# Shadowfear36/SegHiero

Measured on AMD Instinct MI355X. Metric: images/sec at 512x512 (ResNet-50 2-level), full train step, higher is better.
Workload: dtype f32 (convolutions: exact 3-way bf16 split of every fp32 operand, 6 bf16 MFMA products, f32 accumulate; rest plain f32)

## Files before the change

seghiero_amd/csrc/bn_elementwise.hip:

```cpp
#include "common.h"
#include <stdlib.h>

static inline unsigned grid_for(long long work_items, int block = 256, int cap = 4096) {
    long long g = sh_cdiv(work_items, block);
    if (g > cap) g = cap;
    if (g < 1) g = 1;
    return (unsigned)g;
}

__global__ __launch_bounds__(256) void nchw_to_nhwc_kernel(const float* __restrict__ x, float* __restrict__ y,
                                                           int C, long long HW, int Cpad, long long total) {
    for (long long i = (long long)blockIdx.x * 256 + threadIdx.x; i < total; i += (long long)gridDim.x * 256) {
        const int c = (int)(i % Cpad);
        const long long q = i / Cpad, hw = q % HW, n = q / HW;
        y[i] = c < C ? x[(n * C + c) * HW + hw] : 0.f;
    }
}
__global__ __launch_bounds__(256) void nhwc_to_nchw_kernel(const float* __restrict__ x, float* __restrict__ y,
                                                           int C, long long HW, int Cpad, long long total) {
    for (long long i = (long long)blockIdx.x * 256 + threadIdx.x; i < total; i += (long long)gridDim.x * 256) {
        const long long hw = i % HW, q = i / HW;
        const int c = (int)(q % C);
        const long long n = q / C;
        y[i] = x[(n * HW + hw) * Cpad + c];
// ... 268 lines not shown
        !beta || !running_mean || !running_var || !mean || !invstd || !scale || !shift) return SH_EINVAL;
    if ((long long)n_partials != sh_cdiv((long long)count, rows_per_partial) || (partials_ld != 0 && partials_ld < C)) return SH_EINVAL;
    BnMultiTab T;
    for (int i = 0; i < k; ++i) {
        if (!mean[i] || !invstd[i] || !scale[i] || !shift[i] || partials_col[i] < 0 || (running_mean[i] == nullptr) != (running_var[i] == nullptr))
            return SH_EINVAL;
        T.gamma[i] = gamma[i]; T.beta[i] = beta[i]; T.rm[i] = running_mean[i]; T.rv[i] = running_var[i];
        T.mean[i] = mean[i]; T.invstd[i] = invstd[i]; T.scale[i] = scale[i]; T.shift[i] = shift[i];
        T.wmul[i] = chan_mul ? chan_mul[i] : nullptr; T.isy[i] = isy ? isy[i] : nullptr; T.col[i] = partials_col[i];
        if (T.wmul[i] && chan_stride <= 0) return SH_EINVAL;
    }
    dim3 grid((unsigned)sh_cdiv(C, 4), (unsigned)k);
    bn_finalize_multi_kernel<<<grid, 256, 0, (hipStream_t)stream>>>(partials, n_partials, C, count, eps, momentum, rows_per_partial, partials_ld,
                                                                   chan_stride, T);
    return sh_launch_status();
}
extern "C" int sh_bn_finalize_scaled(const float* partials, int n_partials, int C, double count, const float* chan_mul, int chan_stride,
                                     const float* gamma, const float* beta, float eps, float momentum, float* running_mean,
                                     float* running_var, float* mean, float* invstd, float* scale, float* shift, float* isy,
                                     int rows_per_partial, void* stream) {
    if (!partials || n_partials <= 0 || C <= 0 || count <= 0 || !chan_mul || chan_stride <= 0 || !mean || !invstd || !scale || !shift || !isy ||
        rows_per_partial <= 0) return SH_EINVAL;
    if ((long long)n_partials != sh_cdiv((long long)count, rows_per_partial)) return SH_EINVAL;
    if ((running_mean == nullptr) != (running_var == nullptr)) return SH_EINVAL;
    bn_finalize_kernel<256><<<(unsigned)sh_cdiv(C, 4), 256, 0, (hipStream_t)stream>>>(
        partials, n_partials, C, count, gamma, beta, eps, momentum, running_mean, running_var, mean, invstd, scale, shift, rows_per_partial,
        0, chan_mul, chan_stride, isy);
    return sh_launch_status();
}
__global__ __launch_bounds__(64) void dw_center_wgrad_kernel(const float* __restrict__ dgamma, const float* __restrict__ gamma,
                                                             const float* __restrict__ isy, const float* __restrict__ w, float eps,
                                                             float* __restrict__ dw, int C, const float* __restrict__ g, long long ldg,
                                                             const float* __restrict__ x, long long ldx, const float* __restrict__ mean_x,
                                                             long long M) {
    const int c = blockIdx.x, t = threadIdx.x;
    const float wc = w[(long long)c * 9 + 4];
    const float gm = gamma ? gamma[c] : 1.f;
    float v = 0.f;
    if (wc != 0.f) v = gm * dgamma[c] * eps * isy[c] * isy[c] / wc;
    else if (g != nullptr) {
        const float mu = mean_x[c];
        double s = 0.0;
        for (long long m = t; m < M; m += 64) s += (double)g[m * ldg + c] * (double)(x[m * ldx + c] - mu);
#pragma unroll
        for (int o = 32; o > 0; o >>= 1) s += __shfl_xor(s, o, 64);
        v = (float)((double)gm * (double)isy[c] * s);
    }
    if (t < 9) dw[(long long)c * 9 + t] = t == 4 ? v : 0.f;
}
extern "C" int sh_dw_center_wgrad(const float* dgamma, const float* gamma, const float* isy, const float* w, float eps, float* dw, int C,
                                  const float* g, int ldg, const float* x, int ldx, const float* mean_x, int64_t M, void* stream) {
    if (!dgamma || !isy || !w || !dw || C <= 0) return SH_EINVAL;
    if (g && (!x || !mean_x || ldg < C || ldx < C || M <= 0)) return SH_EINVAL;
    dw_center_wgrad_kernel<<<(unsigned)C, 64, 0, (hipStream_t)stream>>>(dgamma, gamma, isy, w, eps, dw, C, g, ldg, x, ldx, mean_x, M);
    return sh_launch_status();
}

__global__ __launch_bounds__(256) void bn_eval_coefs_kernel(const float* gamma, const float* beta, const float* rm,
                                                            const float* rv, float eps, int C, float* scale, float* shift) {
    const int c = blockIdx.x * 256 + threadIdx.x;
    if (c >= C) return;
    const float is = 1.0f / sqrtf(rv[c] + eps);
    const float sc = (gamma ? gamma[c] : 1.f) * is;
    scale[c] = sc;
    shift[c] = (beta ? beta[c] : 0.f) - rm[c] * sc;
}
extern "C" int sh_bn_eval_coefs(const float* gamma, const float* beta, const float* running_mean,
                                const float* running_var, float eps, int C, float* scale, float* shift, void* stream) {
    if (!running_mean || !running_var || !scale || !shift || C <= 0) return SH_EINVAL;
    bn_eval_coefs_kernel<<<(unsigned)sh_cdiv(C, 256), 256, 0, (hipStream_t)stream>>>(gamma, beta, running_mean, running_var, eps, C, scale, shift);
    return sh_launch_status();
}

#define STAT_ROWS 256
template <int KIND>
__global__ __launch_bounds__(256) void channel_partials_kernel(const float* __restrict__ y, long long ldy,
                                                               const float* __restrict__ dout, long long lddo,
                                                               const float* __restrict__ out, long long ldo,
                                                               const float* __restrict__ mean, const float* __restrict__ invstd,
                                                               const float* __restrict__ scale, const float* __restrict__ shift,
                                                               float* __restrict__ partials, long long M, int C, int relu) {
    __shared__ float red[2][4][64];
    const int t = threadIdx.x, cl = t & 63, g = t >> 6;
    const int c = blockIdx.y * 64 + cl;
    const long long rbeg = (long long)blockIdx.x * STAT_ROWS;
    const long long rend = rbeg + STAT_ROWS < M ? rbeg + STAT_ROWS : M;
    float s = 0.f, q = 0.f;
    if (c < C) {
        float mu = 0.f, is = 0.f, sc = 0.f, sh = 0.f;
        if (KIND == 1) { mu = mean[c]; is = invstd[c]; if (relu == 2) { sc = scale[c]; sh = shift[c]; } }
        for (long long r = rbeg + g; r < rend; r += 4) {
            if (KIND == 0) {
                const float v = y[r * ldy + c];
                s += v; q += v * v;
            } else {
                float gv = dout[r * lddo + c];
                const float yv = y[r * ldy + c];
                if (relu == 1 && !(out[r * ldo + c] > 0.f)) gv = 0.f;
                if (relu == 2 && !(yv * sc + sh > 0.f)) gv = 0.f;
                const float xh = (yv - mu) * is;
                s += gv; q += gv * xh;
            }
        }
    }
    if (KIND == 0) {
        float n = 0.f, mean = 0.f, m2 = 0.f;
        if (c < C)
            for (long long r = rbeg + g; r < rend; r += 4) {
                const float v = y[r * ldy + c];
                n += 1.f;
                const float d = v - mean;
                mean += d / n;
                m2 += d * (v - mean);
            }
        red[0][g][cl] = n * mean; red[1][g][cl] = m2;
        __shared__ float cnt[4][64];
        cnt[g][cl] = n;
        __syncthreads();
        if (t < 64) {
            const int ch = blockIdx.y * 64 + t;
            if (ch < C) {
                float N = cnt[0][t], S = red[0][0][t], Q = red[1][0][t];
#pragma unroll
                for (int k = 1; k < 4; ++k) {
                    const float nb = cnt[k][t], sb = red[0][k][t];
                    if (nb > 0.f) {
                        if (N > 0.f) { const float dm = S / N - sb / nb; Q += red[1][k][t] + dm * dm * N * nb / (N + nb); }
                        else Q = red[1][k][t];
                        N += nb; S += sb;
                    }
                }
                partials[((long long)blockIdx.x * 2 + 0) * C + ch] = S;
                partials[((long long)blockIdx.x * 2 + 1) * C + ch] = Q;
            }
        }
        return;
    }
    red[0][g][cl] = s; red[1][g][cl] = q;
    __syncthreads();
    if (t < 128) {
        const int st = t >> 6, cc = t & 63, ch = blockIdx.y * 64 + cc;
        if (ch < C)
            partials[((long long)blockIdx.x * 2 + st) * C + ch] = (red[st][0][cc] + red[st][1][cc]) + (red[st][2][cc] + red[st][3][cc]);
    }
}
__global__ __launch_bounds__(256) void channel_stats_v4_kernel(const float* __restrict__ y, long long ldy, float* __restrict__ partials,
                                                               long long M, int C) {
    __shared__ float red[16][64];
    __shared__ float colmean[64];
    const int t = threadIdx.x, cq = t & 15, rl = t >> 4;
    const unsigned nch = (unsigned)((C + 63) / 64), rb = blockIdx.x / nch, cb = blockIdx.x % nch;
    const int c = cb * 64 + cq * 4;
    const long long rbeg = (long long)rb * STAT_ROWS;
    const long long left = M - rbeg;
    const float nvalid = (float)(left < STAT_ROWS ? left : STAT_ROWS);
    f32x4 v[STAT_ROWS / 16];
    f32x4 s = {0.f, 0.f, 0.f, 0.f};
#pragma unroll
    for (int k = 0; k < STAT_ROWS / 16; ++k) {
        const long long r = rbeg + rl + 16 * k;
        v[k] = (c < C && r < M) ? ld4(y + r * ldy + c) : f32x4{0.f, 0.f, 0.f, 0.f};
        s += v[k];
    }
#pragma unroll
    for (int j = 0; j < 4; ++j) red[rl][cq * 4 + j] = s[j];
    __syncthreads();
    float colsum = 0.f;
    if (t < 64) {
#pragma unroll
        for (int k = 0; k < 16; ++k) colsum += red[k][t];
        colmean[t] = colsum / nvalid;
    }
    __syncthreads();
    const f32x4 mu = ld4(&colmean[cq * 4]);
    f32x4 q = {0.f, 0.f, 0.f, 0.f};
#pragma unroll
    for (int k = 0; k < STAT_ROWS / 16; ++k)
        if (rbeg + rl + 16 * k < M) { const f32x4 d = v[k] - mu; q += d * d; }
#pragma unroll
    for (int j = 0; j < 4; ++j) red[rl][cq * 4 + j] = q[j];
    __syncthreads();
    if (t < 64 && cb * 64 + t < C) {
        float m2 = 0.f;
#pragma unroll
        for (int k = 0; k < 16; ++k) m2 += red[k][t];
        partials[((long long)rb * 2 + 0) * C + cb * 64 + t] = colsum;
        partials[((long long)rb * 2 + 1) * C + cb * 64 + t] = m2;
    }
}
extern "C" int sh_stats_partials_count(int64_t M) { return (int)sh_cdiv(M, STAT_ROWS); }
extern "C" int sh_stats_tile_rows(void) { return STAT_ROWS; }
extern "C" int sh_channel_stats(const float* y, int ldy, int64_t M, int C, float* partials, void* stream) {
    if (!y || !partials || M <= 0 || C <= 0 || ldy < C) return SH_EINVAL;
    dim3 grid((unsigned)sh_cdiv(M, STAT_ROWS), (unsigned)sh_cdiv(C, 64));
    if ((C & 3) == 0 && (ldy & 3) == 0 && ((uintptr_t)y & 15) == 0)
        channel_stats_v4_kernel<<<grid.x * grid.y, 256, 0, (hipStream_t)stream>>>(y, ldy, partials, M, C);
    else
        channel_partials_kernel<0><<<grid, 256, 0, (hipStream_t)stream>>>(y, ldy, nullptr, 0, nullptr, 0, nullptr, nullptr, nullptr, nullptr, partials, M, C, 0);
    return sh_launch_status();
}
__global__ __launch_bounds__(256) void bn_bwd_partials_v4_kernel(const float* __restrict__ y, long long ldy,
                                                                 const float* __restrict__ dout, long long lddo,
                                                                 const float* __restrict__ out, long long ldo,
                                                                 const float* __restrict__ mean, const float* __restrict__ invstd,
                                                                 const float* __restrict__ scale, const float* __restrict__ shift,
                                                                 float* __restrict__ partials, long long M, int C, int relu,
                                                                 float* __restrict__ g_out, long long ldg, int af) {
    __shared__ float red[2][16][64];
    const int t = threadIdx.x, cq = t & 15, rl = t >> 4;
    const unsigned nch = (unsigned)((C + 63) / 64), rb = blockIdx.x / nch, cb = blockIdx.x % nch;
    const int c = cb * 64 + cq * 4;
    const long long rbeg = (long long)rb * STAT_ROWS;
    f32x4 s = {0.f, 0.f, 0.f, 0.f}, q = {0.f, 0.f, 0.f, 0.f};
    if (c < C) {
        const f32x4 mu = ld4(mean + c), is = ld4(invstd + c);
        f32x4 sc = {0.f, 0.f, 0.f, 0.f}, sh = sc;
        if (relu == 2) { sc = ld4(scale + c); sh = ld4(shift + c); }
#pragma unroll 4
        for (int k = 0; k < STAT_ROWS / 16; ++k) {
            const long long r = rbeg + rl + 16 * k;
            if (r < M) {
                f32x4 g = lda4(dout, r * lddo + c, af & 4);
                const f32x4 yv = lda4(y, r * ldy + c, af & 1);
                if (relu == 1) {
                    const f32x4 o = lda4(out, r * ldo + c, af & 2);
#pragma unroll
                    for (int j = 0; j < 4; ++j) g[j] = o[j] > 0.f ? g[j] : 0.f;
                } else if (relu == 2) {
                    const f32x4 o = yv * sc + sh;
#pragma unroll
                    for (int j = 0; j < 4; ++j) g[j] = o[j] > 0.f ? g[j] : 0.f;
                } else if (relu == 3) {
                    const f32x4 o = quad_mask_load(out, r * ldo + (c >> 2));
#pragma unroll
                    for (int j = 0; j < 4; ++j) g[j] = o[j] > 0.f ? g[j] : 0.f;
                }
                s += g;
                q += g * ((yv - mu) * is);
                if (g_out) sta4(g_out, r * ldg + c, g, af & 8);
            }
        }
    }
#pragma unroll
    for (int j = 0; j < 4; ++j) { red[0][rl][cq * 4 + j] = s[j]; red[1][rl][cq * 4 + j] = q[j]; }
    __syncthreads();
    if (t < 128) {
        const int st = t >> 6, cc = t & 63, ch = cb * 64 + cc;
        if (ch < C) {
            float a = 0.f;
#pragma unroll
            for (int k = 0; k < 16; ++k) a += red[st][k][cc];
            partials[((long long)rb * 2 + st) * C + ch] = a;
        }
    }
}
extern "C" int sh_bn_bwd_reduce(const float* dout, int lddo, const float* out, int ldo, const float* y, int ldy,
                                const float* mean, const float* invstd, const float* scale, const float* shift, float* partials,
                                int64_t M, int C, int relu, float* g_out, int ldg, int act_flags, void* stream) {
    if (!dout || !y || !mean || !invstd || !partials || M <= 0 || C <= 0 || lddo < C || ldy < C) return SH_EINVAL;
    if (g_out && (ldg < C || (ldg & 3) || ((uintptr_t)g_out & 15))) return SH_EINVAL;
    if (relu < 0 || relu > 3 || (relu == 1 && (!out || ldo < C)) || (relu == 2 && (!scale || !shift)) || (relu == 3 && (!out || ldo * 4 < C))) return SH_EINVAL;
    dim3 grid((unsigned)sh_cdiv(M, STAT_ROWS), (unsigned)sh_cdiv(C, 64));
    const bool v4 = (C & 3) == 0 && ((lddo | ldy | (relu == 1 ? ldo : 0)) & 3) == 0 && ((uintptr_t)dout & 15) == 0 && ((uintptr_t)y & 15) == 0 &&
                    (relu != 1 || ((uintptr_t)out & 15) == 0) && ((uintptr_t)mean & 15) == 0 && ((uintptr_t)invstd & 15) == 0 &&
                    (relu != 2 || ((((uintptr_t)scale | (uintptr_t)shift) & 15) == 0));
    if (v4) bn_bwd_partials_v4_kernel<<<grid.x * grid.y, 256, 0, (hipStream_t)stream>>>(y, ldy, dout, lddo, out, ldo, mean, invstd, scale, shift, partials, M, C, relu, g_out, ldg, act_flags);
    else if (g_out || act_flags || relu == 3) return SH_EUNSUPPORTED;
    else channel_partials_kernel<1><<<grid, 256, 0, (hipStream_t)stream>>>(y, ldy, dout, lddo, out, ldo, mean, invstd, scale, shift, partials, M, C, relu);
    return sh_launch_status();
}

__device__ __forceinline__ void bn_bwd_lin(float* lin, int C, int c, float ga, float is, float mu, float c1, float c2) {
    const float A = ga * is;
    lin[c] = A; lin[C + c] = -(A * is) * c2; lin[2 * C + c] = mu; lin[3 * C + c] = -A * c1;
}
template <int NT>
__global__ __launch_bounds__(NT) void bn_bwd_finalize_kernel(const float* __restrict__ partials, int P, int C,
                                                              const float* __restrict__ gamma, const float* __restrict__ invstd,
                                                              double count, float* dgamma, float* dbeta, float* c1, float* c2,
                                                              const float* __restrict__ mean, float* __restrict__ lin) {
    const int cpre = blockIdx.x * 4 + threadIdx.x;
    float ga = 1.f, is = 0.f, mu = 0.f;
    if (lin && threadIdx.x < 4 && cpre < C) { if (gamma) ga = gamma[cpre]; is = invstd[cpre]; mu = mean[cpre]; }
    reduce_partials_4ch<NT>(partials, P, C, blockIdx.x * 4, 0, 0, [&](int c, double s, double q) {
        if (dbeta) dbeta[c] = (float)s;
        if (dgamma) dgamma[c] = (float)q;
        const float f1 = (float)(s / count), f2 = (float)(q / count);
        c1[c] = f1;
        c2[c] = f2;
        if (lin) bn_bwd_lin(lin, C, c, ga, is, mu, f1, f2);
    });
}
extern "C" int sh_bn_bwd_finalize(const float* partials, int n_partials, int C, const float* gamma, const float* invstd,
                                  double count, float* dgamma, float* dbeta, float* c1, float* c2, const float* mean, float* lin,
                                  void* stream) {
    if (!partials || n_partials <= 0 || C <= 0 || count <= 0 || !c1 || !c2 || (lin && (!mean || !invstd))) return SH_EINVAL;
    if (n_partials >= 1024)
        bn_bwd_finalize_kernel<1024><<<(unsigned)sh_cdiv(C, 4), 1024, 0, (hipStream_t)stream>>>(partials, n_partials, C, gamma, invstd, count, dgamma, dbeta, c1, c2, mean, lin);
    else
        bn_bwd_finalize_kernel<256><<<(unsigned)sh_cdiv(C, 4), 256, 0, (hipStream_t)stream>>>(partials, n_partials, C, gamma, invstd, count, dgamma, dbeta, c1, c2, mean, lin);
    return sh_launch_status();
}

#define EW_ROWS 16
template <int V>
__global__ __launch_bounds__(256) void bn_act_kernel(const float* __restrict__ y, long long ldy, const float* __restrict__ scale,
                                                     const float* __restrict__ shift, const float* __restrict__ res, long long ldr,
                                                     float* __restrict__ out, long long ldo, long long M, int C, int relu,
                                                     const float* __restrict__ rscale, const float* __restrict__ rshift, int af,
                                                     unsigned char* __restrict__ qmask) {
    const int cv = C / V;
    for (long long m0 = (long long)blockIdx.x * EW_ROWS; m0 < M; m0 += (long long)gridDim.x * EW_ROWS)
    for (int e = threadIdx.x, tot = (int)((M - m0 < EW_ROWS ? M - m0 : EW_ROWS)) * cv; e < tot; e += 256) {
        const int r = e / cv;
        const long long m = m0 + r;
        const int c = (e - r * cv) * V;
        if (V == 8) {
            const sh_f8 yv = lda8(y, m * ldy + c, af & 1);
            sh_f8 v;
            v.lo = yv.lo * ld4(scale + c) + ld4(shift + c); v.hi = yv.hi * ld4(scale + c + 4) + ld4(shift + c + 4);
            if (res) {
                sh_f8 r = lda8(res, m * ldr + c, af & 2);
                if (rscale) { r.lo = r.lo * ld4(rscale + c) + ld4(rshift + c); r.hi = r.hi * ld4(rscale + c + 4) + ld4(rshift + c + 4); }
                v.lo += r.lo; v.hi += r.hi;
            }
            if (relu) {
#pragma unroll
                for (int j = 0; j < 4; ++j) { v.lo[j] = fmaxf(v.lo[j], 0.f); v.hi[j] = fmaxf(v.hi[j], 0.f); }
            }
            sta8(out, m * ldo + c, v, af & 4);
            if (qmask) *reinterpret_cast<unsigned short*>(qmask + m * (C / 4) + (c >> 2)) = (unsigned short)(quad_mask_bits(v.lo) | (quad_mask_bits(v.hi) << 8));
        } else if (V == 4) {
            f32x4 v = lda4(y, m * ldy + c, af & 1) * ld4(scale + c) + ld4(shift + c);
            if (res) {
                f32x4 r = lda4(res, m * ldr + c, af & 2);
                if (rscale) r = r * ld4(rscale + c) + ld4(rshift + c);
                v += r;
            }
            if (relu) { v[0] = fmaxf(v[0], 0.f); v[1] = fmaxf(v[1], 0.f); v[2] = fmaxf(v[2], 0.f); v[3] = fmaxf(v[3], 0.f); }
            sta4(out, m * ldo + c, v, af & 4);
            if (qmask) qmask[m * cv + (c >> 2)] = (unsigned char)quad_mask_bits(v);
        } else {
            float v = y[m * ldy + c] * scale[c] + shift[c];
            if (res) v += rscale ? res[m * ldr + c] * rscale[c] + rshift[c] : res[m * ldr + c];
            if (relu) v = fmaxf(v, 0.f);
            out[m * ldo + c] = v;
        }
    }
}
static inline unsigned rows_grid(long long M, int cv) {
    (void)cv;
    long long g = sh_cdiv(M, EW_ROWS);
    if (g > 8192) g = 8192;
    return (unsigned)(g < 1 ? 1 : g);
}
static inline bool vec4_ok(int C, long long a, long long b = 0, long long c = 0, long long d = 0, long long e = 0) {
    return (C & 3) == 0 && ((a | b | c | d | e) & 3) == 0;
}
static inline bool ptr16(const void* p) { return ((uintptr_t)p & 15) == 0; }
static inline bool ew8_on() { const char* e = getenv("SEGHIERO_EW8"); return !(e && e[0] == '0'); }

extern "C" int sh_bn_act(const float* y, int ldy, const float* scale, const float* shift, const float* residual, int ldr,
                         const float* res_scale, const float* res_shift, float* out, int ldo, int64_t M, int C, int relu, uint8_t* relu_mask,
                         int act_flags, void* stream) {
    if (!y || !scale || !shift || !out || M <= 0 || C <= 0 || ldy < C || ldo < C) return SH_EINVAL;
    if (residual && ldr < C) return SH_EINVAL;
    if ((res_scale == nullptr) != (res_shift == nullptr) || (res_scale && !residual)) return SH_EINVAL;
    const bool v4 = vec4_ok(C, ldy, ldo, residual ? ldr : 0) && ptr16(y) && ptr16(out) && ptr16(scale) && ptr16(shift) && (!residual || ptr16(residual)) &&
                    (!res_scale || (ptr16(res_scale) && ptr16(res_shift)));
    if ((act_flags || relu_mask) && !v4) return SH_EUNSUPPORTED;
    const bool v8 = v4 && ew8_on() && (act_flags & 1) && (C & 7) == 0 && ((ldy | ldo | (residual ? ldr : 0)) & 7) == 0 && (!relu_mask || ((uintptr_t)relu_mask & 1) == 0);
    if (v8) bn_act_kernel<8><<<rows_grid(M, C / 8), 256, 0, (hipStream_t)stream>>>(y, ldy, scale, shift, residual, ldr, out, ldo, M, C, relu, res_scale, res_shift, act_flags, relu_mask);
    else if (v4) bn_act_kernel<4><<<rows_grid(M, C / 4), 256, 0, (hipStream_t)stream>>>(y, ldy, scale, shift, residual, ldr, out, ldo, M, C, relu, res_scale, res_shift, act_flags, relu_mask);
    else bn_act_kernel<1><<<rows_grid(M, C), 256, 0, (hipStream_t)stream>>>(y, ldy, scale, shift, residual, ldr, out, ldo, M, C, relu, res_scale, res_shift, 0, nullptr);
    return sh_launch_status();
}

template <int V>
__global__ __launch_bounds__(256) void bn_bwd_apply_kernel(const float* __restrict__ dout, long long lddo, const float* __restrict__ out,
                                                           long long ldo, const float* __restrict__ y, long long ldy,
                                                           const float* __restrict__ mean, const float* __restrict__ invstd,
                                                           const float* __restrict__ scale, const float* __restrict__ shift,
                                                           const float* __restrict__ gamma, const float* __restrict__ c1,
                                                           const float* __restrict__ c2, float* __restrict__ dy, long long lddy,
                                                           float* __restrict__ dres, long long lddres, long long M, int C, int relu, int af) {
    const int cv = C / V;
    for (long long m0 = (long long)blockIdx.x * EW_ROWS; m0 < M; m0 += (long long)gridDim.x * EW_ROWS)
    for (int e = threadIdx.x, tot = (int)((M - m0 < EW_ROWS ? M - m0 : EW_ROWS)) * cv; e < tot; e += 256) {
        const int r = e / cv;
        const long long m = m0 + r;
        const int c = (e - r * cv) * V;
        if (V == 8) {
            sh_f8 g8 = lda8(dout, m * lddo + c, af & 4);
            const sh_f8 y8 = lda8(y, m * ldy + c, af & 1);
            sh_f8 o8 = sh_f8{f32x4{1.f, 1.f, 1.f, 1.f}, f32x4{1.f, 1.f, 1.f, 1.f}};
            if (relu == 1) o8 = lda8(out, m * ldo + c, af & 2);
            else if (relu == 2) { o8.lo = y8.lo * ld4(scale + c) + ld4(shift + c); o8.hi = y8.hi * ld4(scale + c + 4) + ld4(shift + c + 4); }
            else if (relu == 3) { o8.lo = quad_mask_load(out, m * ldo + (c >> 2)); o8.hi = quad_mask_load(out, m * ldo + (c >> 2) + 1); }
            if (relu) {
#pragma unroll
                for (int j = 0; j < 4; ++j) { if (!(o8.lo[j] > 0.f)) g8.lo[j] = 0.f; if (!(o8.hi[j] > 0.f)) g8.hi[j] = 0.f; }
            }
            sh_f8 r8;
            {
                const f32x4 is = ld4(invstd + c), xh = (y8.lo - ld4(mean + c)) * is;
                f32x4 ga = {1.f, 1.f, 1.f, 1.f};
                if (gamma) ga = ld4(gamma + c);
                r8.lo = ga * is * (g8.lo - ld4(c1 + c) - xh * ld4(c2 + c));
            }
            {
                const f32x4 is = ld4(invstd + c + 4), xh = (y8.hi - ld4(mean + c + 4)) * is;
                f32x4 ga = {1.f, 1.f, 1.f, 1.f};
                if (gamma) ga = ld4(gamma + c + 4);
                r8.hi = ga * is * (g8.hi - ld4(c1 + c + 4) - xh * ld4(c2 + c + 4));
            }
            sta8(dy, m * lddy + c, r8, af & 8);
            if (dres) sta8(dres, m * lddres + c, g8, af & 16);
        } else if (V == 4) {
            f32x4 g = lda4(dout, m * lddo + c, af & 4);
            const f32x4 yv = lda4(y, m * ldy + c, af & 1);
            if (relu == 1) {
                const f32x4 o = lda4(out, m * ldo + c, af & 2);
#pragma unroll
                for (int j = 0; j < 4; ++j) if (!(o[j] > 0.f)) g[j] = 0.f;
            } else if (relu == 2) {
                const f32x4 o = yv * ld4(scale + c) + ld4(shift + c);
#pragma unroll
                for (int j = 0; j < 4; ++j) if (!(o[j] > 0.f)) g[j] = 0.f;
            } else if (relu == 3) {
                const f32x4 o = quad_mask_load(out, m * ldo + (c >> 2));
#pragma unroll
                for (int j = 0; j < 4; ++j) if (!(o[j] > 0.f)) g[j] = 0.f;
            }
            const f32x4 is = ld4(invstd + c);
            const f32x4 xh = (yv - ld4(mean + c)) * is;
            f32x4 ga = {1.f, 1.f, 1.f, 1.f};
            if (gamma) ga = ld4(gamma + c);
            const f32x4 r = ga * is * (g - ld4(c1 + c) - xh * ld4(c2 + c));
            sta4(dy, m * lddy + c, r, af & 8);
            if (dres) sta4(dres, m * lddres + c, g, af & 16);
        } else {
            float g = dout[m * lddo + c];
            const float yv = y[m * ldy + c];
            if (relu == 1 && !(out[m * ldo + c] > 0.f)) g = 0.f;
            if (relu == 2 && !(yv * scale[c] + shift[c] > 0.f)) g = 0.f;
            const float is = invstd[c];
            const float xh = (yv - mean[c]) * is;
            dy[m * lddy + c] = (gamma ? gamma[c] : 1.f) * is * (g - c1[c] - xh * c2[c]);
            if (dres) dres[m * lddres + c] = g;
        }
    }
}
extern "C" int sh_bn_bwd_apply(const float* dout, int lddo, const float* out, int ldo, const float* y, int ldy,
                               const float* mean, const float* invstd, const float* scale, const float* shift, const float* gamma,
                               const float* c1, const float* c2, float* dy, int lddy, float* dres, int lddres, int64_t M, int C, int relu,
                               int act_flags, void* stream) {
    if (!dout || !y || !mean || !invstd || !c1 || !c2 || !dy || M <= 0 || C <= 0 || lddo < C || ldy < C || lddy < C) return SH_EINVAL;
    if (relu < 0 || relu > 3 || (relu == 1 && (!out || ldo < C)) || (relu == 2 && (!scale || !shift)) || (relu == 3 && (!out || ldo * 4 < C))) return SH_EINVAL;
    if (dres && lddres < C) return SH_EINVAL;
    const bool v4 = vec4_ok(C, lddo, ldy, lddy, relu == 1 ? ldo : 0, dres ? lddres : 0) && ptr16(dout) && ptr16(y) && ptr16(dy) &&
                    ptr16(mean) && ptr16(invstd) && ptr16(c1) && ptr16(c2) && (!gamma || ptr16(gamma)) && (relu != 1 || ptr16(out)) &&
                    (relu != 2 || (ptr16(scale) && ptr16(shift))) && (!dres || ptr16(dres));
    if ((act_flags || relu == 3) && !v4) return SH_EUNSUPPORTED;
    const bool v8 = v4 && ew8_on() && (act_flags & 1) && (C & 7) == 0 && ((lddo | ldy | lddy | (relu == 1 ? ldo : 0) | (dres ? lddres : 0)) & 7) == 0 && (relu != 3 || (ldo & 1) == 0);
    if (v8) bn_bwd_apply_kernel<8><<<rows_grid(M, C / 8), 256, 0, (hipStream_t)stream>>>(dout, lddo, out, ldo, y, ldy, mean, invstd, scale, shift, gamma, c1, c2, dy, lddy, dres, lddres, M, C, relu, act_flags);
    else if (v4) bn_bwd_apply_kernel<4><<<rows_grid(M, C / 4), 256, 0, (hipStream_t)stream>>>(dout, lddo, out, ldo, y, ldy, mean, invstd, scale, shift, gamma, c1, c2, dy, lddy, dres, lddres, M, C, relu, act_flags);
    else bn_bwd_apply_kernel<1><<<rows_grid(M, C), 256, 0, (hipStream_t)stream>>>(dout, lddo, out, ldo, y, ldy, mean, invstd, scale, shift, gamma, c1, c2, dy, lddy, dres, lddres, M, C, relu, 0);
    return sh_launch_status();
}

__global__ __launch_bounds__(256) void bn_reduce_partials_kernel(const float* __restrict__ partials, int P, int C, int R, long long M,
                                                                 double* __restrict__ sq) {
    if (blockIdx.x == 0 && threadIdx.x == 0) sq[2 * C] = (double)M;
    reduce_partials_4ch(partials, P, C, blockIdx.x * 4, R, M, [&](int c, double s, double q) { sq[c] = s; sq[C + c] = q; });
}
extern "C" int sh_bn_reduce_partials(const float* partials, int n_partials, int C, double count, int rows_per_partial, double* sq,
                                     void* stream) {
    if (!partials || !sq || n_partials <= 0 || C <= 0 || rows_per_partial < 0) return SH_EINVAL;
    bn_reduce_partials_kernel<<<(unsigned)sh_cdiv(C, 4), 256, 0, (hipStream_t)stream>>>(partials, n_partials, C, rows_per_partial,
                                                                                       (long long)count, sq);
    return sh_launch_status();
}
__global__ __launch_bounds__(256) void bn_finalize_sq_kernel(const double* __restrict__ sq, int C, const float* __restrict__ gamma,
                                                             const float* __restrict__ beta, float eps, float momentum, float* running_mean,
                                                             float* running_var, float* mean, float* invstd, float* scale, float* shift) {
    const int c = blockIdx.x * 256 + threadIdx.x;
    if (c >= C) return;
    const double count = sq[2 * C];
    const double mu = sq[c] / count;
    double var = sq[C + c] / count - mu * mu;
    if (var < 0) var = 0;
    const float fmu = (float)mu, is = 1.0f / sqrtf((float)var + eps);
    mean[c] = fmu; invstd[c] = is;
    const float sc = (gamma ? gamma[c] : 1.f) * is;
    scale[c] = sc; shift[c] = (beta ? beta[c] : 0.f) - fmu * sc;
    if (running_mean) {
        const double unbiased = count > 1 ? var * (count / (count - 1.0)) : var;
        running_mean[c] = (1.f - momentum) * running_mean[c] + momentum * fmu;
        running_var[c] = (1.f - momentum) * running_var[c] + momentum * (float)unbiased;
    }
}
extern "C" int sh_bn_finalize_sq(const double* sq, int C, const float* gamma, const float* beta, float eps, float momentum,
                                 float* running_mean, float* running_var, float* mean, float* invstd, float* scale, float* shift,
                                 void* stream) {
    if (!sq || C <= 0 || !mean || !invstd || !scale || !shift) return SH_EINVAL;
    bn_finalize_sq_kernel<<<(unsigned)sh_cdiv(C, 256), 256, 0, (hipStream_t)stream>>>(sq, C, gamma, beta, eps, momentum, running_mean,
                                                                                      running_var, mean, invstd, scale, shift);
    return sh_launch_status();
}
__global__ __launch_bounds__(256) void bn_bwd_finalize_sq_kernel(const double* __restrict__ local_sq, const double* __restrict__ global_sq, int C,
                                                                 float* dgamma, float* dbeta, float* c1, float* c2, const float* gamma,
                                                                 const float* invstd, const float* mean, float* lin) {
    const int c = blockIdx.x * 256 + threadIdx.x;
    if (c >= C) return;
    const double count = global_sq[2 * C];
    if (dbeta) dbeta[c] = (float)local_sq[c];
    if (dgamma) dgamma[c] = (float)local_sq[C + c];
    const float f1 = (float)(global_sq[c] / count), f2 = (float)(global_sq[C + c] / count);
    c1[c] = f1;
    c2[c] = f2;
    if (lin) bn_bwd_lin(lin, C, c, gamma ? gamma[c] : 1.f, invstd[c], mean[c], f1, f2);
}
extern "C" int sh_bn_bwd_finalize_sq(const double* local_sq, const double* global_sq, int C, float* dgamma, float* dbeta,
                                     float* c1, float* c2, const float* gamma, const float* invstd, const float* mean, float* lin, void* stream) {
    if (!local_sq || !global_sq || C <= 0 || !c1 || !c2 || (lin && (!mean || !invstd))) return SH_EINVAL;
    bn_bwd_finalize_sq_kernel<<<(unsigned)sh_cdiv(C, 256), 256, 0, (hipStream_t)stream>>>(local_sq, global_sq, C, dgamma, dbeta, c1, c2, gamma, invstd, mean, lin);
    return sh_launch_status();
}
```

seghiero_amd/csrc/common.h:

```cpp
#pragma once
#include <hip/hip_runtime.h>
#include <stdint.h>
#include "../../include/seghiero_hip.h"

typedef float f32x4 __attribute__((ext_vector_type(4)));
typedef float f32x16 __attribute__((ext_vector_type(16)));

#define SH_WAVE 64

static inline int sh_launch_status() {
    hipError_t e = hipGetLastError();
    return e == hipSuccess ? SH_OK : SH_ELAUNCH;
}

static inline int64_t sh_cdiv(int64_t a, int64_t b) { return (a + b - 1) / b; }

__device__ __forceinline__ float wave_sum(float v) {
#pragma unroll
    for (int o = 32; o > 0; o >>= 1) v += __shfl_xor(v, o, 64);
    return v;
}
__device__ __forceinline__ double wave_sum_d(double v) {
#pragma unroll
    for (int o = 32; o > 0; o >>= 1) v += __shfl_xor(v, o, 64);
    return v;
}

__device__ __forceinline__ unsigned xcd_remap(unsigned bid, unsigned nblk) {
    const unsigned q = nblk >> 3, r = nblk & 7u, xcd = bid & 7u, loc = bid >> 3;
    const unsigned base = xcd < r ? xcd * (q + 1) : r * (q + 1) + (xcd - r) * q;
    return base + loc;
}

__device__ __forceinline__ f32x4 ld4(const float* p) { return *reinterpret_cast<const f32x4*>(p); }
__device__ __forceinline__ void st4(float* p, f32x4 v) { *reinterpret_cast<f32x4*>(p) = v; }

typedef unsigned int sh_u32x2 __attribute__((ext_vector_type(2)));
__device__ __forceinline__ f32x4 bf16x4_to_f32(sh_u32x2 v) {
    return f32x4{__uint_as_float(v[0] << 16), __uint_as_float(v[0] & 0xffff0000u), __uint_as_float(v[1] << 16), __uint_as_float(v[1] & 0xffff0000u)};
}
__device__ __forceinline__ unsigned f32_to_bf16_rne(float f) {
    const unsigned u = __float_as_uint(f);
    return (f != f) ? ((u >> 16) | 0x40u) : ((u + 0x7fffu + ((u >> 16) & 1u)) >> 16);
}
__device__ __forceinline__ sh_u32x2 f32_to_bf16x4(f32x4 v) {
    return sh_u32x2{f32_to_bf16_rne(v[0]) | (f32_to_bf16_rne(v[1]) << 16), f32_to_bf16_rne(v[2]) | (f32_to_bf16_rne(v[3]) << 16)};
}
__device__ __forceinline__ f32x4 lda4(const float* base, long long idx, int bf) {
    if (bf) return bf16x4_to_f32(*reinterpret_cast<const sh_u32x2*>(reinterpret_cast<const unsigned short*>(base) + idx));
    return ld4(base + idx);
}
__device__ __forceinline__ unsigned quad_mask_bits(f32x4 v) {
    return (v[0] > 0.f ? 1u : 0u) | (v[1] > 0.f ? 2u : 0u) | (v[2] > 0.f ? 4u : 0u) | (v[3] > 0.f ? 8u : 0u);
}
__device__ __forceinline__ f32x4 quad_mask_load(const void* base, long long byte_idx) {
    const unsigned b = reinterpret_cast<const unsigned char*>(base)[byte_idx];
    return f32x4{(b & 1u) ? 1.f : 0.f, (b & 2u) ? 1.f : 0.f, (b & 4u) ? 1.f : 0.f, (b & 8u) ? 1.f : 0.f};
}
__device__ __forceinline__ void sta4(float* base, long long idx, f32x4 v, int bf) {
    if (bf) *reinterpret_cast<sh_u32x2*>(reinterpret_cast<unsigned short*>(base) + idx) = f32_to_bf16x4(v);
    else st4(base + idx, v);
}

struct sh_f8 { f32x4 lo, hi; };
typedef unsigned int sh_u32x4 __attribute__((ext_vector_type(4)));
__device__ __forceinline__ sh_f8 lda8(const float* base, long long idx, int bf) {
    sh_f8 r;
    if (bf) {
        const sh_u32x4 v = *reinterpret_cast<const sh_u32x4*>(reinterpret_cast<const unsigned short*>(base) + idx);
        r.lo = bf16x4_to_f32(sh_u32x2{v[0], v[1]}); r.hi = bf16x4_to_f32(sh_u32x2{v[2], v[3]});
    } else { r.lo = ld4(base + idx); r.hi = ld4(base + idx + 4); }
    return r;
}
__device__ __forceinline__ void sta8(float* base, long long idx, const sh_f8& v, int bf) {
    if (bf) {
        const sh_u32x2 a = f32_to_bf16x4(v.lo), b = f32_to_bf16x4(v.hi);
        *reinterpret_cast<sh_u32x4*>(reinterpret_cast<unsigned short*>(base) + idx) = sh_u32x4{a[0], a[1], b[0], b[1]};
    } else { st4(base + idx, v.lo); st4(base + idx + 4, v.hi); }
}
```

Measured before the change: 506.7.

## Restructure BN elementwise kernels into 2D channel-tiled, row-unrolled, templated variants

Rewrites the BN forward activation and BN backward apply kernels so each thread owns a fixed channel vector and walks rows with a 4-way unrolled batch of loads issued before compute. Per-channel coefficients (scale, shift, mean, invstd, c1, c2, gamma) are loaded once into registers instead of per element, and the residual and relu modes plus the bf16 flag become template parameters so inner-loop branches compile away. The aim is to cut per-element div/mod indexing and redundant coefficient loads and to raise memory-level parallelism in these bandwidth-bound kernels. The cost is more template instantiations, higher register use, and a clamped duplicate load for the tail rows.

```diff
diff --git a/seghiero_amd/csrc/bn_elementwise.hip b/seghiero_amd/csrc/bn_elementwise.hip
--- a/seghiero_amd/csrc/bn_elementwise.hip
+++ b/seghiero_amd/csrc/bn_elementwise.hip
@@ -594,54 +594,113 @@
     return sh_launch_status();
 }
 
+#define EW_U 4
+#define EW_GRID 16384
+struct EwGeom { int w, ty, np; unsigned grid; };
+static inline EwGeom ew_geom(long long M, int cv) {
+    EwGeom g;
+    g.np = (int)sh_cdiv(cv, 256); g.w = (int)sh_cdiv(cv, g.np); g.ty = 256 / g.w;
+    long long gx = EW_GRID / g.np;
+    const long long slabs = sh_cdiv(M, (long long)g.ty * EW_U);
+    if (gx > slabs) gx = slabs;
+    if (gx < 1) gx = 1;
+    g.grid = (unsigned)(gx * g.np);
+    return g;
+}
+template <int V>
+__device__ __forceinline__ bool ew_thread(int cv, EwGeom G, int& c, long long& m0, long long& mstep) {
+    const int t = threadIdx.x, tr = t / G.w, tx = t - tr * G.w;
+    const unsigned piece = blockIdx.x % (unsigned)G.np, slab = blockIdx.x / (unsigned)G.np, nslab = gridDim.x / (unsigned)G.np;
+    const int cx = (int)piece * G.w + tx;
+    c = cx * V;
+    m0 = (long long)slab * (G.ty * EW_U) + tr;
+    mstep = (long long)nslab * (G.ty * EW_U);
+    return tr < G.ty && cx < cv;
+}
+template <int V> struct ew_vec { f32x4 q[V / 4]; };
+template <int V> __device__ __forceinline__ ew_vec<V> ew_ld(const float* base, long long idx, int bf) {
+    ew_vec<V> r;
+    if constexpr (V == 8) { const sh_f8 v = lda8(base, idx, bf); r.q[0] = v.lo; r.q[1] = v.hi; }
+    else r.q[0] = lda4(base, idx, bf);
+    return r;
+}
+template <int V> __device__ __forceinline__ void ew_st(float* base, long long idx, const ew_vec<V>& v, int bf) {
+    if constexpr (V == 8) sta8(base, idx, sh_f8{v.q[0], v.q[1]}, bf);
+    else sta4(base, idx, v.q[0], bf);
+}
+template <int V> __device__ __forceinline__ ew_vec<V> ew_coef(const float* p, int c) {
+    ew_vec<V> r;
+#pragma unroll
+    for (int h = 0; h < V / 4; ++h) r.q[h] = ld4(p + c + 4 * h);
+    return r;
+}
+
 #define EW_ROWS 16
-template <int V>
+template <int V, int RES, bool BF>
 __global__ __launch_bounds__(256) void bn_act_kernel(const float* __restrict__ y, long long ldy, const float* __restrict__ scale,
                                                      const float* __restrict__ shift, const float* __restrict__ res, long long ldr,
                                                      float* __restrict__ out, long long ldo, long long M, int C, int relu,
                                                      const float* __restrict__ rscale, const float* __restrict__ rshift, int af,
-                                                     unsigned char* __restrict__ qmask) {
-    const int cv = C / V;
+                                                     unsigned char* __restrict__ qmask, EwGeom G) {
+    constexpr int H = V / 4;
+    int c;
+    long long m0, mstep;
+    if (!ew_thread<V>(C / V, G, c, m0, mstep)) return;
+    if (!BF) af = 0;
+    const ew_vec<V> sc = ew_coef<V>(scale, c), sh = ew_coef<V>(shift, c);
+    ew_vec<V> rsc = sc, rsh = sh;
+    if (RES == 2) { rsc = ew_coef<V>(rscale, c); rsh = ew_coef<V>(rshift, c); }
+    for (; m0 < M; m0 += mstep) {
+        ew_vec<V> yv[EW_U], rv[EW_U];
+#pragma unroll
+        for (int u = 0; u < EW_U; ++u) {
+            const long long m = m0 + u * G.ty, mc = m < M ? m : M - 1;
+            yv[u] = ew_ld<V>(y, mc * ldy + c, af & 1);
+            if (RES) rv[u] = ew_ld<V>(res, mc * ldr + c, af & 2);
+        }
+#pragma unroll
+        for (int u = 0; u < EW_U; ++u) {
+            const long long m = m0 + u * G.ty;
+            if (m < M) {
+                ew_vec<V> v;
+#pragma unroll
+                for (int h = 0; h < H; ++h) {
+                    v.q[h] = yv[u].q[h] * sc.q[h] + sh.q[h];
+                    if (RES) {
+                        f32x4 r = rv[u].q[h];
+                        if (RES == 2) r = r * rsc.q[h] + rsh.q[h];
+                        v.q[h] += r;
+                    }
+                    if (relu) {
+#pragma unroll
+                        for (int j = 0; j < 4; ++j) v.q[h][j] = fmaxf(v.q[h][j], 0.f);
+                    }
+                }
+                ew_st<V>(out, m * ldo + c, v, af & 4);
+                if (qmask) {
+                    if constexpr (V == 8) *reinterpret_cast<unsigned short*>(qmask + m * (C / 4) + (c >> 2)) = (unsigned short)(quad_mask_bits(v.q[0]) | (quad_mask_bits(v.q[1]) << 8));
+                    else qmask[m * (C / 4) + (c >> 2)] = (unsigned char)quad_mask_bits(v.q[0]);
+                }
+            }
+        }
+    }
+}
+__global__ __launch_bounds__(256) void bn_act_scalar_kernel(const float* __restrict__ y, long long ldy, const float* __restrict__ scale,
+                                                            const float* __restrict__ shift, const float* __restrict__ res, long long ldr,
+                                                            float* __restrict__ out, long long ldo, long long M, int C, int relu,
+                                                            const float* __restrict__ rscale, const float* __restrict__ rshift) {
     for (long long m0 = (long long)blockIdx.x * EW_ROWS; m0 < M; m0 += (long long)gridDim.x * EW_ROWS)
-    for (int e = threadIdx.x, tot = (int)((M - m0 < EW_ROWS ? M - m0 : EW_ROWS)) * cv; e < tot; e += 256) {
-        const int r = e / cv;
+    for (int e = threadIdx.x, tot = (int)((M - m0 < EW_ROWS ? M - m0 : EW_ROWS)) * C; e < tot; e += 256) {
+        const int r = e / C;
         const long long m = m0 + r;
-        const int c = (e - r * cv) * V;
-        if (V == 8) {
-            const sh_f8 yv = lda8(y, m * ldy + c, af & 1);
-            sh_f8 v;
-            v.lo = yv.lo * ld4(scale + c) + ld4(shift + c); v.hi = yv.hi * ld4(scale + c + 4) + ld4(shift + c + 4);
-            if (res) {
-                sh_f8 r = lda8(res, m * ldr + c, af & 2);
-                if (rscale) { r.lo = r.lo * ld4(rscale + c) + ld4(rshift + c); r.hi = r.hi * ld4(rscale + c + 4) + ld4(rshift + c + 4); }
-                v.lo += r.lo; v.hi += r.hi;
-            }
-            if (relu) {
-#pragma unroll
-                for (int j = 0; j < 4; ++j) { v.lo[j] = fmaxf(v.lo[j], 0.f); v.hi[j] = fmaxf(v.hi[j], 0.f); }
-            }
-            sta8(out, m * ldo + c, v, af & 4);
-            if (qmask) *reinterpret_cast<unsigned short*>(qmask + m * (C / 4) + (c >> 2)) = (unsigned short)(quad_mask_bits(v.lo) | (quad_mask_bits(v.hi) << 8));
-        } else if (V == 4) {
-            f32x4 v = lda4(y, m * ldy + c, af & 1) * ld4(scale + c) + ld4(shift + c);
-            if (res) {
-                f32x4 r = lda4(res, m * ldr + c, af & 2);
-                if (rscale) r = r * ld4(rscale + c) + ld4(rshift + c);
-                v += r;
-            }
-            if (relu) { v[0] = fmaxf(v[0], 0.f); v[1] = fmaxf(v[1], 0.f); v[2] = fmaxf(v[2], 0.f); v[3] = fmaxf(v[3], 0.f); }
-            sta4(out, m * ldo + c, v, af & 4);
-            if (qmask) qmask[m * cv + (c >> 2)] = (unsigned char)quad_mask_bits(v);
-        } else {
-            float v = y[m * ldy + c] * scale[c] + shift[c];
-            if (res) v += rscale ? res[m * ldr + c] * rscale[c] + rshift[c] : res[m * ldr + c];
-            if (relu) v = fmaxf(v, 0.f);
-            out[m * ldo + c] = v;
-        }
-    }
-}
-static inline unsigned rows_grid(long long M, int cv) {
-    (void)cv;
+        const int c = e - r * C;
+        float v = y[m * ldy + c] * scale[c] + shift[c];
+        if (res) v += rscale ? res[m * ldr + c] * rscale[c] + rshift[c] : res[m * ldr + c];
+        if (relu) v = fmaxf(v, 0.f);
+        out[m * ldo + c] = v;
+    }
+}
+static inline unsigned rows_grid(long long M) {
     long long g = sh_cdiv(M, EW_ROWS);
     if (g > 8192) g = 8192;
     return (unsigned)(g < 1 ? 1 : g);
@@ -652,6 +711,12 @@
 static inline bool ptr16(const void* p) { return ((uintptr_t)p & 15) == 0; }
 static inline bool ew8_on() { const char* e = getenv("SEGHIERO_EW8"); return !(e && e[0] == '0'); }
 
+template <int V, bool BF, typename... A>
+static inline void launch_bn_act(int res_form, const EwGeom& g, hipStream_t st, A... args) {
+    if (res_form == 0) bn_act_kernel<V, 0, BF><<<g.grid, 256, 0, st>>>(args..., g);
+    else if (res_form == 1) bn_act_kernel<V, 1, BF><<<g.grid, 256, 0, st>>>(args..., g);
+    else bn_act_kernel<V, 2, BF><<<g.grid, 256, 0, st>>>(args..., g);
+}
 extern "C" int sh_bn_act(const float* y, int ldy, const float* scale, const float* shift, const float* residual, int ldr,
                          const float* res_scale, const float* res_shift, float* out, int ldo, int64_t M, int C, int relu, uint8_t* relu_mask,
                          int act_flags, void* stream) {
@@ -662,86 +727,99 @@
                     (!res_scale || (ptr16(res_scale) && ptr16(res_shift)));
     if ((act_flags || relu_mask) && !v4) return SH_EUNSUPPORTED;
     const bool v8 = v4 && ew8_on() && (act_flags & 1) && (C & 7) == 0 && ((ldy | ldo | (residual ? ldr : 0)) & 7) == 0 && (!relu_mask || ((uintptr_t)relu_mask & 1) == 0);
-    if (v8) bn_act_kernel<8><<<rows_grid(M, C / 8), 256, 0, (hipStream_t)stream>>>(y, ldy, scale, shift, residual, ldr, out, ldo, M, C, relu, res_scale, res_shift, act_flags, relu_mask);
-    else if (v4) bn_act_kernel<4><<<rows_grid(M, C / 4), 256, 0, (hipStream_t)stream>>>(y, ldy, scale, shift, residual, ldr, out, ldo, M, C, relu, res_scale, res_shift, act_flags, relu_mask);
-    else bn_act_kernel<1><<<rows_grid(M, C), 256, 0, (hipStream_t)stream>>>(y, ldy, scale, shift, residual, ldr, out, ldo, M, C, relu, res_scale, res_shift, 0, nullptr);
-    return sh_launch_status();
-}
-
-template <int V>
+    const hipStream_t st = (hipStream_t)stream;
+    const int res_form = !residual ? 0 : (res_scale ? 2 : 1);
+    const long long Ml = M;
+    if (v8) launch_bn_act<8, true>(res_form, ew_geom(M, C / 8), st, y, (long long)ldy, scale, shift, residual, (long long)ldr, out, (long long)ldo, Ml, C, relu, res_scale, res_shift, act_flags, relu_mask);
+    else if (v4 && act_flags) launch_bn_act<4, true>(res_form, ew_geom(M, C / 4), st, y, (long long)ldy, scale, shift, residual, (long long)ldr, out, (long long)ldo, Ml, C, relu, res_scale, res_shift, act_flags, relu_mask);
+    else if (v4) launch_bn_act<4, false>(res_form, ew_geom(M, C / 4), st, y, (long long)ldy, scale, shift, residual, (long long)ldr, out, (long long)ldo, Ml, C, relu, res_scale, res_shift, 0, relu_mask);
+    else bn_act_scalar_kernel<<<rows_grid(M), 256, 0, st>>>(y, ldy, scale, shift, residual, ldr, out, ldo, M, C, relu, res_scale, res_shift);
+    return sh_launch_status();
+}
+
+template <int V, int RM, bool BF>
 __global__ __launch_bounds__(256) void bn_bwd_apply_kernel(const float* __restrict__ dout, long long lddo, const float* __restrict__ out,
                                                            long long ldo, const float* __restrict__ y, long long ldy,
                                                            const float* __restrict__ mean, const float* __restrict__ invstd,
                                                            const float* __restrict__ scale, const float* __restrict__ shift,
                                                            const float* __restrict__ gamma, const float* __restrict__ c1,
                                                            const float* __restrict__ c2, float* __restrict__ dy, long long lddy,
-                                                           float* __restrict__ dres, long long lddres, long long M, int C, int relu, int af) {
-    const int cv = C / V;
+                                                           float* __restrict__ dres, long long lddres, long long M, int C, int af, EwGeom G) {
+    constexpr int H = V / 4;
+    int c;
+    long long m0, mstep;
+    if (!ew_thread<V>(C / V, G, c, m0, mstep)) return;
+    if (!BF) af = 0;
+    const ew_vec<V> is = ew_coef<V>(invstd, c), mu = ew_coef<V>(mean, c), k1 = ew_coef<V>(c1, c), k2 = ew_coef<V>(c2, c);
+    ew_vec<V> ga, sc = is, sh = is;
+#pragma unroll
+    for (int h = 0; h < H; ++h) ga.q[h] = f32x4{1.f, 1.f, 1.f, 1.f};
+    if (gamma) ga = ew_coef<V>(gamma, c);
+    if (RM == 2) { sc = ew_coef<V>(scale, c); sh = ew_coef<V>(shift, c); }
+    for (; m0 < M; m0 += mstep) {
+        ew_vec<V> g[EW_U], yv[EW_U], o[EW_U];
+        unsigned mb[EW_U][H];
+#pragma unroll
+        for (int u = 0; u < EW_U; ++u) {
+            const long long m = m0 + u * G.ty, mc = m < M ? m : M - 1;
+            g[u] = ew_ld<V>(dout, mc * lddo + c, af & 4);
+            yv[u] = ew_ld<V>(y, mc * ldy + c, af & 1);
+            if (RM == 1) o[u] = ew_ld<V>(out, mc * ldo + c, af & 2);
+            if (RM == 3) {
+#pragma unroll
+                for (int h = 0; h < H; ++h) mb[u][h] = quad_mask_byte(out, mc * ldo + (c >> 2) + h);
+            }
+        }
+#pragma unroll
+        for (int u = 0; u < EW_U; ++u) {
+            const long long m = m0 + u * G.ty;
+            if (m < M) {
+                ew_vec<V> r;
+#pragma unroll
+                for (int h = 0; h < H; ++h) {
+                    if (RM == 2) o[u].q[h] = yv[u].q[h] * sc.q[h] + sh.q[h];
+                    if (RM == 3) o[u].q[h] = quad_mask_unpack(mb[u][h]);
+                    if (RM) {
+#pragma unroll
+                        for (int j = 0; j < 4; ++j) if (!(o[u].q[h][j] > 0.f)) g[u].q[h][j] = 0.f;
+                    }
+                    const f32x4 xh = (yv[u].q[h] - mu.q[h]) * is.q[h];
+                    r.q[h] = ga.q[h] * is.q[h] * (g[u].q[h] - k1.q[h] - xh * k2.q[h]);
+                }
+                ew_st<V>(dy, m * lddy + c, r, af & 8);
+                if (dres) ew_st<V>(dres, m * lddres + c, g[u], af & 16);
+            }
+        }
+    }
+}
+__global__ __launch_bounds__(256) void bn_bwd_apply_scalar_kernel(const float* __restrict__ dout, long long lddo, const float* __restrict__ out,
+                                                                  long long ldo, const float* __restrict__ y, long long ldy,
+                                                                  const float* __restrict__ mean, const float* __restrict__ invstd,
+                                                                  const float* __restrict__ scale, const float* __restrict__ shift,
+                                                                  const float* __restrict__ gamma, const float* __restrict__ c1,
+                                                                  const float* __restrict__ c2, float* __restrict__ dy, long long lddy,
+                                                                  float* __restrict__ dres, long long lddres, long long M, int C, int relu) {
     for (long long m0 = (long long)blockIdx.x * EW_ROWS; m0 < M; m0 += (long long)gridDim.x * EW_ROWS)
-    for (int e = threadIdx.x, tot = (int)((M - m0 < EW_ROWS ? M - m0 : EW_ROWS)) * cv; e < tot; e += 256) {
-        const int r = e / cv;
+    for (int e = threadIdx.x, tot = (int)((M - m0 < EW_ROWS ? M - m0 : EW_ROWS)) * C; e < tot; e += 256) {
+        const int r = e / C;
         const long long m = m0 + r;
-        const int c = (e - r * cv) * V;
-        if (V == 8) {
-            sh_f8 g8 = lda8(dout, m * lddo + c, af & 4);
-            const sh_f8 y8 = lda8(y, m * ldy + c, af & 1);
-            sh_f8 o8 = sh_f8{f32x4{1.f, 1.f, 1.f, 1.f}, f32x4{1.f, 1.f, 1.f, 1.f}};
-            if (relu == 1) o8 = lda8(out, m * ldo + c, af & 2);
-            else if (relu == 2) { o8.lo = y8.lo * ld4(scale + c) + ld4(shift + c); o8.hi = y8.hi * ld4(scale + c + 4) + ld4(shift + c + 4); }
-            else if (relu == 3) { o8.lo = quad_mask_load(out, m * ldo + (c >> 2)); o8.hi = quad_mask_load(out, m * ldo + (c >> 2) + 1); }
-            if (relu) {
-#pragma unroll
-                for (int j = 0; j < 4; ++j) { if (!(o8.lo[j] > 0.f)) g8.lo[j] = 0.f; if (!(o8.hi[j] > 0.f)) g8.hi[j] = 0.f; }
-            }
-            sh_f8 r8;
-            {
-                const f32x4 is = ld4(invstd + c), xh = (y8.lo - ld4(mean + c)) * is;
-                f32x4 ga = {1.f, 1.f, 1.f, 1.f};
-                if (gamma) ga = ld4(gamma + c);
-                r8.lo = ga * is * (g8.lo - ld4(c1 + c) - xh * ld4(c2 + c));
-            }
-            {
-                const f32x4 is = ld4(invstd + c + 4), xh = (y8.hi - ld4(mean + c + 4)) * is;
-                f32x4 ga = {1.f, 1.f, 1.f, 1.f};
-                if (gamma) ga = ld4(gamma + c + 4);
-                r8.hi = ga * is * (g8.hi - ld4(c1 + c + 4) - xh * ld4(c2 + c + 4));
-            }
-            sta8(dy, m * lddy + c, r8, af & 8);
-            if (dres) sta8(dres, m * lddres + c, g8, af & 16);
-        } else if (V == 4) {
-            f32x4 g = lda4(dout, m * lddo + c, af & 4);
-            const f32x4 yv = lda4(y, m * ldy + c, af & 1);
-            if (relu == 1) {
-                const f32x4 o = lda4(out, m * ldo + c, af & 2);
-#pragma unroll
-                for (int j = 0; j < 4; ++j) if (!(o[j] > 0.f)) g[j] = 0.f;
-            } else if (relu == 2) {
-                const f32x4 o = yv * ld4(scale + c) + ld4(shift + c);
-#pragma unroll
-                for (int j = 0; j < 4; ++j) if (!(o[j] > 0.f)) g[j] = 0.f;
-            } else if (relu == 3) {
-                const f32x4 o = quad_mask_load(out, m * ldo + (c >> 2));
-#pragma unroll
-                for (int j = 0; j < 4; ++j) if (!(o[j] > 0.f)) g[j] = 0.f;
-            }
-            const f32x4 is = ld4(invstd + c);
-            const f32x4 xh = (yv - ld4(mean + c)) * is;
-            f32x4 ga = {1.f, 1.f, 1.f, 1.f};
-            if (gamma) ga = ld4(gamma + c);
-            const f32x4 r = ga * is * (g - ld4(c1 + c) - xh * ld4(c2 + c));
-            sta4(dy, m * lddy + c, r, af & 8);
-            if (dres) sta4(dres, m * lddres + c, g, af & 16);
-        } else {
-            float g = dout[m * lddo + c];
-            const float yv = y[m * ldy + c];
-            if (relu == 1 && !(out[m * ldo + c] > 0.f)) g = 0.f;
-            if (relu == 2 && !(yv * scale[c] + shift[c] > 0.f)) g = 0.f;
-            const float is = invstd[c];
-            const float xh = (yv - mean[c]) * is;
-            dy[m * lddy + c] = (gamma ? gamma[c] : 1.f) * is * (g - c1[c] - xh * c2[c]);
-            if (dres) dres[m * lddres + c] = g;
-        }
-    }
+        const int c = e - r * C;
+        float g = dout[m * lddo + c];
+        const float yv = y[m * ldy + c];
+        if (relu == 1 && !(out[m * ldo + c] > 0.f)) g = 0.f;
+        if (relu == 2 && !(yv * scale[c] + shift[c] > 0.f)) g = 0.f;
+        const float is = invstd[c];
+        const float xh = (yv - mean[c]) * is;
+        dy[m * lddy + c] = (gamma ? gamma[c] : 1.f) * is * (g - c1[c] - xh * c2[c]);
+        if (dres) dres[m * lddres + c] = g;
+    }
+}
+template <int V, bool BF, typename... A>
+static inline void launch_bn_bwd_apply(int relu, const EwGeom& g, hipStream_t st, A... args) {
+    if (relu == 0) bn_bwd_apply_kernel<V, 0, BF><<<g.grid, 256, 0, st>>>(args..., g);
+    else if (relu == 1) bn_bwd_apply_kernel<V, 1, BF><<<g.grid, 256, 0, st>>>(args..., g);
+    else if (relu == 2) bn_bwd_apply_kernel<V, 2, BF><<<g.grid, 256, 0, st>>>(args..., g);
+    else bn_bwd_apply_kernel<V, 3, BF><<<g.grid, 256, 0, st>>>(args..., g);
 }
 extern "C" int sh_bn_bwd_apply(const float* dout, int lddo, const float* out, int ldo, const float* y, int ldy,
                                const float* mean, const float* invstd, const float* scale, const float* shift, const float* gamma,
@@ -755,9 +833,12 @@
                     (relu != 2 || (ptr16(scale) && ptr16(shift))) && (!dres || ptr16(dres));
     if ((act_flags || relu == 3) && !v4) return SH_EUNSUPPORTED;
     const bool v8 = v4 && ew8_on() && (act_flags & 1) && (C & 7) == 0 && ((lddo | ldy | lddy | (relu == 1 ? ldo : 0) | (dres ? lddres : 0)) & 7) == 0 && (relu != 3 || (ldo & 1) == 0);
-    if (v8) bn_bwd_apply_kernel<8><<<rows_grid(M, C / 8), 256, 0, (hipStream_t)stream>>>(dout, lddo, out, ldo, y, ldy, mean, invstd, scale, shift, gamma, c1, c2, dy, lddy, dres, lddres, M, C, relu, act_flags);
-    else if (v4) bn_bwd_apply_kernel<4><<<rows_grid(M, C / 4), 256, 0, (hipStream_t)stream>>>(dout, lddo, out, ldo, y, ldy, mean, invstd, scale, shift, gamma, c1, c2, dy, lddy, dres, lddres, M, C, relu, act_flags);
-    else bn_bwd_apply_kernel<1><<<rows_grid(M, C), 256, 0, (hipStream_t)stream>>>(dout, lddo, out, ldo, y, ldy, mean, invstd, scale, shift, gamma, c1, c2, dy, lddy, dres, lddres, M, C, relu, 0);
+    const hipStream_t st = (hipStream_t)stream;
+    const long long Ml = M;
+    if (v8) launch_bn_bwd_apply<8, true>(relu, ew_geom(M, C / 8), st, dout, (long long)lddo, out, (long long)ldo, y, (long long)ldy, mean, invstd, scale, shift, gamma, c1, c2, dy, (long long)lddy, dres, (long long)lddres, Ml, C, act_flags);
+    else if (v4 && act_flags) launch_bn_bwd_apply<4, true>(relu, ew_geom(M, C / 4), st, dout, (long long)lddo, out, (long long)ldo, y, (long long)ldy, mean, invstd, scale, shift, gamma, c1, c2, dy, (long long)lddy, dres, (long long)lddres, Ml, C, act_flags);
+    else if (v4) launch_bn_bwd_apply<4, false>(relu, ew_geom(M, C / 4), st, dout, (long long)lddo, out, (long long)ldo, y, (long long)ldy, mean, invstd, scale, shift, gamma, c1, c2, dy, (long long)lddy, dres, (long long)lddres, Ml, C, 0);
+    else bn_bwd_apply_scalar_kernel<<<rows_grid(M), 256, 0, st>>>(dout, lddo, out, ldo, y, ldy, mean, invstd, scale, shift, gamma, c1, c2, dy, lddy, dres, lddres, M, C, relu);
     return sh_launch_status();
 }
 
diff --git a/seghiero_amd/csrc/common.h b/seghiero_amd/csrc/common.h
--- a/seghiero_amd/csrc/common.h
+++ b/seghiero_amd/csrc/common.h
@@ -53,10 +53,11 @@
 __device__ __forceinline__ unsigned quad_mask_bits(f32x4 v) {
     return (v[0] > 0.f ? 1u : 0u) | (v[1] > 0.f ? 2u : 0u) | (v[2] > 0.f ? 4u : 0u) | (v[3] > 0.f ? 8u : 0u);
 }
-__device__ __forceinline__ f32x4 quad_mask_load(const void* base, long long byte_idx) {
-    const unsigned b = reinterpret_cast<const unsigned char*>(base)[byte_idx];
+__device__ __forceinline__ unsigned quad_mask_byte(const void* base, long long byte_idx) { return reinterpret_cast<const unsigned char*>(base)[byte_idx]; }
+__device__ __forceinline__ f32x4 quad_mask_unpack(unsigned b) {
     return f32x4{(b & 1u) ? 1.f : 0.f, (b & 2u) ? 1.f : 0.f, (b & 4u) ? 1.f : 0.f, (b & 8u) ? 1.f : 0.f};
 }
+__device__ __forceinline__ f32x4 quad_mask_load(const void* base, long long byte_idx) { return quad_mask_unpack(quad_mask_byte(base, byte_idx)); }
 __device__ __forceinline__ void sta4(float* base, long long idx, f32x4 v, int bf) {
     if (bf) *reinterpret_cast<sh_u32x2*>(reinterpret_cast<unsigned short*>(base) + idx) = f32_to_bf16x4(v);
     else st4(base + idx, v);
```

New measurement: 511.6 (median of 6 runs). About the same (+1.0%).
